# termuxinator/html5-canvas-raytracer

Measured on AMD Instinct MI355X. Metric: Mpixel/s, higher is better.
Workload: dtype f64; 1 GPU; cfg3: h8 scene (8 spheres, 2 lights, depth 3, supersample 1) at 3840x2160; SCENE, CAMERA AND LAUNCH TABLE RESIDENT (a static frame rendered again and again: cold_frame / new_camera_every_step are the other cases); one launch per frame; kernel=fma

## Files before the change

html5-canvas-raytracer_amd/csrc/rt_kernel.hip:

```cpp

#include <hip/hip_runtime.h>
#include <math.h>
#include <stdint.h>

#include "rt_device.h"
#include "rt_block.h"
#include "rt_wide.h"

#ifndef RT_STRICT
#define RT_STRICT 0
#endif
#if RT_STRICT
#define RT_LAUNCH_NAME rt_launch_trace_strict
#define RT_SCRATCH_NAME rt_scratch_trace_strict
#else
#define RT_LAUNCH_NAME rt_launch_trace_fast
#define RT_SCRATCH_NAME rt_scratch_trace_fast
#endif

#ifndef RT_WAVES_PER_EU
#define RT_WAVES_PER_EU 2
#endif

#define RT_INF __builtin_inf()

namespace {

#include "rt_literal.h"
#include "rt_kernel_math.h"
#include "rt_kernel_entry.h"
#include "rt_kernel_tables.h"
#include "rt_kernel_trace.h"

#if !RT_STRICT
typedef uint32_t __attribute__((ext_vector_type(4))) rt_px4;
__device__ __forceinline__ void rt_store16(uint32_t *p, rt_px4 v, bool through) {
  if (through) asm volatile("global_store_dwordx4 %0, %1, off sc1\n\ts_nop 1" :: "v"(p), "v"(v) : "memory");
  else *(rt_px4 *)p = v;
}
template <int N>
__device__ __forceinline__ uint32_t rt_row_down(uint32_t x) { return (uint32_t)__builtin_amdgcn_update_dpp(0, (int)x, 0x100 + N, 0xf, 0xf, true); }
#endif

template <bool REFRACT, bool COUNT, bool SS2, bool GRID, bool W1 = false>
__global__ void __launch_bounds__(W1 ? 64 : RT_WG_THREADS, ((REFRACT || !GRID) ? RT_WAVES_PER_EU : (RT_WAVES_PER_EU > 5 ? RT_WAVES_PER_EU : 5))) rt_trace(const rt_launch L) {
  static_assert(!W1 || (!REFRACT && !COUNT && !RT_STRICT), "one-wave workgroups: the reflection-only product variants");
  [[maybe_unused]] constexpr uint32_t WG_WAVES = W1 ? 1u : RT_WG_THREADS / 64u;
  constexpr uint32_t KT = W1 ? 64u : RT_WG_THREADS;
  extern __shared__ double lds_raw[];
#if defined(RT_WAVE_LOG) && !RT_STRICT
  if (unsigned long long *const wl = rt_cold_args()->wave_log; wl != nullptr && (threadIdx.x & 63u) == 0u) {
    unsigned long long *q = wl + ((size_t)(blockIdx.z * gridDim.x + blockIdx.x) * WG_WAVES + (threadIdx.x >> 6)) * 4u;
    q[0] = __builtin_amdgcn_s_memrealtime();
    q[2] = (unsigned long long)__builtin_amdgcn_s_getreg((4u) | (0u << 6) | (31u << 11)) | ((unsigned long long)__builtin_amdgcn_s_getreg((20u) | (0u << 6) | (31u << 11)) << 32);
    q[3] = rt_entry_index<W1>();
  }
#endif
  const uint32_t tid = threadIdx.x;
  const uint32_t mtl_words = L.n_objects * (uint32_t)(sizeof(rt_mtl) / 8);
  const uint32_t tex_words = 16u * 2u;
  const bool cull_lds_on = (!RT_STRICT && !COUNT) ? !GRID : (L.cull_in_lds != 0u);
  const uint32_t cull_words = cull_lds_on ? L.n_objects * 4u : 0u;
  const uint32_t image_words = mtl_words + tex_words + cull_words;
  constexpr bool IMAGE_IN_LDS = RT_STRICT || COUNT || !(GRID && !REFRACT);
  const uint32_t lds_words = IMAGE_IN_LDS ? image_words : 0u;
  const double *__restrict__ image = (const double *)L.lds_image;
  typedef uint32_t __attribute__((ext_vector_type(4))) rt_u4;
  constexpr uint32_t RT_STAGE_PIECES = 3u;
  const uint32_t image_vec = image_words >> 1;
  [[maybe_unused]] rt_u4 piece[RT_STAGE_PIECES];
  [[maybe_unused]] double stage0 = 0.0;
  const auto stage_issue = [&](const uint32_t tid) __attribute__((always_inline)) {
    if constexpr (!IMAGE_IN_LDS) {
    } else if constexpr (GRID || W1) {
      const rt_u4 *__restrict__ image4 = (const rt_u4 *)L.lds_image;
#pragma unroll
      for (uint32_t i = 0; i < RT_STAGE_PIECES; i++) if (i * KT < image_vec) piece[i] = image4[tid + i * KT];
    } else {
      stage0 = (tid < image_words) ? image[tid] : 0.0;
    }
  };
  constexpr bool UNI_OK = W1 && !REFRACT && !COUNT && !RT_STRICT && !(GRID && SS2);
  if constexpr (!UNI_OK) stage_issue(tid);
  const rt_mtl *mtl = IMAGE_IN_LDS ? (const rt_mtl *)lds_raw : (const rt_mtl *)L.lds_image;
  const rt_texture_desc *tex = IMAGE_IN_LDS ? (const rt_texture_desc *)(lds_raw + mtl_words) : (const rt_texture_desc *)((const double *)L.lds_image + mtl_words);
  const rt_geom *cull_lds = (const rt_geom *)(lds_raw + mtl_words + tex_words);
  double *acc = lds_raw + lds_words + tid;
  rt_geom cull0 = rt_geom{0.0, 0.0, 0.0, 0.0};
  if (!cull_lds_on) { const uint32_t lane0 = tid & 63u; cull0 = L.cull[lane0 < L.n_loop ? lane0 : 0u]; }

  const uint32_t lane = tid & 63u;
  const rt_pixel P0 = rt_pixel_of<SS2, W1>(L, tid);
#if !RT_STRICT
  if constexpr (W1 && !REFRACT && !COUNT && !GRID) rt_head_batch(L);
  if (P0.rows_valid == 0u) return;
#endif
  [[maybe_unused]] bool uni_try = false;
  [[maybe_unused]] uint32_t cell = 0u;
  if constexpr (UNI_OK) {
    uni_try = !P0.sky && (P0.cand >> 16) == 1u;
    if constexpr (!GRID) cell = (P0.cell >> rt_wave_of<W1>(tid)) & 0x11u;
#ifdef RT_TESTING
    if (L.no_uniform) uni_try = false;
    if (L.no_cells) cell = 0u;
#endif
    if (!uni_try && !P0.sky) stage_issue(tid);
  }
  double rgb[3];
// ... 31 lines not shown
  const auto stage_finish = [&](const uint32_t tid) __attribute__((always_inline)) {
    if constexpr (!IMAGE_IN_LDS) {
    } else if constexpr (GRID || W1) {
      rt_u4 *lds4 = (rt_u4 *)lds_raw;
      const rt_u4 *__restrict__ image4 = (const rt_u4 *)L.lds_image;
#pragma unroll
      for (uint32_t i = 0; i < RT_STAGE_PIECES; i++) {
        const uint32_t k = tid + i * KT;
        if (i * KT < image_vec && k < image_vec) lds4[k] = piece[i];
      }
      for (uint32_t k = tid + RT_STAGE_PIECES * KT; k < image_vec; k += KT) lds4[k] = image4[k];
    } else {
      if (tid < image_words) lds_raw[tid] = stage0;
      for (uint32_t k = tid + RT_WG_THREADS; k < image_words; k += RT_WG_THREADS) lds_raw[k] = image[k];
    }
  };
  [[maybe_unused]] bool uni_done = false;
  if constexpr (UNI_OK) {
    if (uni_try) {
      uni_done = trace_pixel<REFRACT, COUNT, GRID, SS2, false, W1, true>(L, (const rt_mtl *)L.lds_image, (const rt_texture_desc *)((const double *)L.lds_image + mtl_words), acc,
                                                                         cull_lds, cull0, lane, 0.0, 0.0, 0.0, 0.0, o, ray, rgb, cnt, is_probe, P0.cand | (cell << 24));
      if (!uni_done) {
        uint32_t tid4 = threadIdx.x;
        asm volatile("" : "+v"(tid4));
        stage_issue(tid4);
        stage_finish(tid4);
      }
#ifdef RT_TESTING
      else if (lane == 0u && L.uniform_waves != nullptr) {
        atomicAdd(L.uniform_waves, 1ull);
        if (cell & 1u) atomicAdd(L.uniform_waves + 1, 1ull);
      }
#endif
    }
  }
  if (!uni_done) {
    if (!UNI_OK || !uni_try) stage_finish(tid);
    if constexpr (IMAGE_IN_LDS) __syncthreads();

    const double bw = SS2 ? 15.0 : 7.0, bh = SS2 ? 3.0 : 7.0;
    const double lx = SS2 ? (double)(2u * ((lane >> 2) & 7u) + (sub & 1u)) : (double)(lane & 7u);
    const double ly = SS2 ? (double)(2u * (lane >> 5) + (sub >> 1)) : (double)(lane >> 3);
    double blk_x0 = 0.0, blk_x1 = 0.0, blk_y0 = 0.0, blk_y1 = 0.0;
    if (!UNI_OK || !uni_try) { blk_x0 = d0 - lx; blk_x1 = blk_x0 + bw; blk_y1 = d1 + ly; blk_y0 = blk_y1 - bh; }
    trace_pixel<REFRACT, COUNT, GRID, SS2, false, W1>(L, mtl, tex, acc, cull_lds, cull0, lane, blk_x0, blk_x1, blk_y0, blk_y1, o, ray, rgb, cnt, is_probe, P0.cand);
  }
  }

  uint32_t tid2 = threadIdx.x;
  asm volatile("" : "+v"(tid2));
  const rt_pixel P1 = rt_pixel_of<SS2, W1>(L, tid2);
#if !RT_STRICT
  const uint32_t wide = rt_cold_args()->wide_stores;
  asm volatile("" :: "s"(wide), "s"(L.scatter), "s"(L.rgb24), "s"(L.w), "s"(L.out), "s"(L.frame_stride));
#endif
  const uint32_t frame_i = blockIdx.z;
  const bool valid = P1.valid;
  const uint32_t r8 = to_byte(rgb[0]), g8 = to_byte(rgb[1]), b8 = to_byte(rgb[2]);
#if RT_STRICT
  uint32_t *__restrict__ out = L.scatter ? L.out_frames[frame_i] : L.out + (size_t)frame_i * L.frame_stride;
  const uint32_t orow = L.scatter ? P1.frow : P1.lrow;
#endif
  uint32_t rgbw;
  if (!SS2) rgbw = r8 | (g8 << 8) | (b8 << 16);
  else {
    uint32_t packed = r8 | (g8 << 10) | (b8 << 20);
    packed += __shfl_xor(packed, 1);
    packed += __shfl_xor(packed, 2);
    rgbw = (((packed & 1023u) + 2u) >> 2) | ((((packed >> 10) & 1023u) + 2u) >> 2 << 8) | ((((packed >> 20) & 1023u) + 2u) >> 2 << 16);
  }
#if RT_STRICT
  const uint32_t n_run = 1u;
// ... 258 lines not shown
```

html5-canvas-raytracer_amd/csrc/rt_kernel_entry.h:

```cpp

struct rt_pixel { uint32_t px, trow, frow, lrow, sub, rows_valid, run, cand, cell; bool valid, sky; };
template <bool W1>
__device__ __forceinline__ uint32_t rt_entry_slot(const rt_launch &L) {
  return (blockIdx.x & 7u) * L.order_n8 + (blockIdx.x >> (W1 ? 5 : 3));
}
template <bool W1>
__device__ __forceinline__ uint32_t rt_entry_index() { return W1 ? (((blockIdx.x >> 5) << 3) | (blockIdx.x & 7u)) : blockIdx.x; }
template <bool W1>
__device__ __forceinline__ uint32_t rt_wave_of(uint32_t tid) { return W1 ? ((blockIdx.x >> 3) & 3u) : tid >> 6; }

#if RT_STRICT
template <bool SS2, bool W1 = false>
__device__ __forceinline__ rt_pixel rt_pixel_of(const rt_launch &L, uint32_t tid) {
  const uint32_t wave = tid >> 6, lane = tid & 63u;
  const uint32_t tile_x = blockIdx.x, by = blockIdx.y;
  uint32_t tile_i, row_block;
  if (L.n_tiles == 1u) { tile_i = 0u; row_block = by; }
  else if (L.rb_shift != ~0u) { tile_i = by >> L.rb_shift; row_block = by & ((1u << L.rb_shift) - 1u); }
  else { tile_i = by / L.rb_per_tile; row_block = by - tile_i * L.rb_per_tile; }
  rt_pixel P;
  P.sub = 0u;
  if (!SS2) { P.px = tile_x * RT_TILE_W + wave * 8u + (lane & 7u); P.trow = row_block * RT_TILE_H + (lane >> 3); }
  else { const uint32_t q = lane >> 2; P.sub = lane & 3u; P.px = tile_x * RT_TILE_W + wave * 8u + (q & 7u); P.trow = row_block * 2u + (q >> 3); }
  P.frow = (L.tile_first + tile_i * L.tile_stride) * L.tile_rows + P.trow;
  P.lrow = tile_i * L.tile_rows + P.trow;
  P.valid = (P.px < L.w) && (P.trow < L.tile_rows) && (P.frow < L.h);
  P.rows_valid = 0u;
  P.sky = false; P.run = 1u; P.cand = 0u; P.cell = 0u;
  return P;
}
#else
template <bool SS2, bool W1 = false>
// ... 69 lines not shown
```

html5-canvas-raytracer_amd/csrc/rt_kernel_trace.h:

```cpp

#define RT_PIN() asm volatile("")
#define RT_ROOT(TCA, DISC)                                                                    \
        const double thc_ = rt_sqrt_nn<REFRACT>(DISC);                                                 \
        const double t0_ = (TCA) - thc_, t1_ = (TCA) + thc_;                                  \
        const bool in_ = (t0_ < eps);                                                         \
        const double t_ = in_ ? t1_ : t0_;
#define RT_CAND(IDX, TCA, DISC)                                                               \
      if (!((DISC) < 0.0)) {                                                                  \
        RT_PIN();                                                                             \
        RT_ROOT(TCA, DISC)                                                                    \
        const bool closer_ = (t_ < ht) && !(t_ < eps);              \
        ht = closer_ ? t_ : ht;                                                               \
        hcode = closer_ ? ((int)(2u * (IDX)) + (in_ ? 1 : 0)) : hcode;                        \
      }
#define RT_GENERIC(IDX, G)                                                                    \
      {                                                                                       \
        const v3 Lv_ = mk((G).ox - p.x, (G).oy - p.y, (G).oz - p.z);                          \
        const double tca_ = dot(d, Lv_);                                                      \
        const double disc_ = (G).r2 - (dot(Lv_, Lv_) - tca_ * tca_);                          \
        RT_CAND(IDX, tca_, disc_)                                                             \
      }
#define RT_ANCHORED_DISC(G)                                                                   \
        const double tca_ = d.x * (G).ox + d.y * (G).oy + d.z * (G).oz;                       \
        const double disc_ = __builtin_fma(tca_, tca_, -(G).r2);
// ... 31 lines not shown
          if (!UNI && near_) {                                                                                  \
            RT_PIN();                                                                                             \
            iu = (uint32_t)(XU); iv = (uint32_t)(XV);                    \
            const rt_launch __attribute__((address_space(4))) *K = rt_cold_args();                                \
             \
            float q_here = RT_Q_GET(level);                                                                        \
            if (rt_lvl(level) == 0 && q_here == 0.f) {                   \
              const float ex = (float)(h.x - K->cam_origin[0]), ey = (float)(h.y - K->cam_origin[1]), ez = (float)(h.z - K->cam_origin[2]);   \
              q_here = RT_Q_OF(0.f, __builtin_sqrtf(ex * ex + ey * ey + ez * ez), (float)m.inv_r, __builtin_fabsf((float)dot(d, n)), 0.f);       \
            }                                                                                                     \
            double tol = (K->mark_flags & RT_MARK_ALL) ? 2.0 : K->flag_tol * (double)fmaxf(1.f, q_here * (1.f / RT_Q_FLAT));   \
                          \
            if ((K->mark_flags & (RT_MARK_WEIGHT | RT_MARK_ALL)) == RT_MARK_WEIGHT) {                              \
              double S_ = map_valid ? acc[0] : 1.0;                                                               \
              if constexpr (FOLD_FORWARD && REFRACT) for (int i_ = 0; i_ < sp; i_++) S_ *= (parked[i_].map_valid ? parked[i_].S : 1.0) * parked[i_].a3;   \
              if (__builtin_fabs(S_) * 510.0 < 0.9) tol = -1.0;                                                    \
            }                                                                                                     \
             \
            const bool zf = !(K->mark_flags & RT_MARK_ZERO);                                                       \
            const bool bu = (zf && (FU) == 0.0 && (XU) == 0.0) || (__builtin_fabs((XU) - __builtin_rint(XU)) >= tol);    \
            const bool bv = (zf && (FV) == 0.0 && (XV) == 0.0) || (__builtin_fabs((XV) - __builtin_rint(XV)) >= tol);    \
            if (!(bu & bv)) {                                                                                      \
              uint32_t t3 = threadIdx.x;                                                                          \
              asm volatile("" : "+v"(t3));                                                                        \
              rt_mark_append<SS2>(rt_pixel_of<SS2, W1>(L, t3));                                                        \
            }                                                                                                     \
          }
#endif

#if !RT_STRICT
#define RT_SDISC(G, TC, DISC)                                                                 \
            const double TC = -(sv.x * (G).ox + sv.y * (G).oy + sv.z * (G).oz);               \
            const double DISC = __builtin_fma(TC, TC, -(G).r2);
#define RT_SROOTS(TC, THC, T0, T1) const double T0 = llen - (TC + THC), T1 = llen - (TC - THC);
#else
#define RT_SDISC(G, TC, DISC)                                                                 \
            const v3 Lv_ = mk((G).ox - h.x, (G).oy - h.y, (G).oz - h.z);                      \
            const double TC = dot(sv, Lv_);                                                   \
            const double DISC = (G).r2 - (dot(Lv_, Lv_) - TC * TC);
#define RT_SROOTS(TC, THC, T0, T1) const double T0 = TC - THC, T1 = TC + THC;
#endif
#define RT_SHADOW(J, G)                                                                       \
            {                                                                                 \
              const bool other_ = ((int)(J) != hi);                                           \
              if (COUNT && other_ && !blocked) tests++;                                       \
              RT_SDISC(G, tc_, disc_)                                                         \
// ... 24 lines not shown
                  li = (oa4_ != 0.0) ? rt_div(li, oa4_) : 0.0;                              \
                }                                                                           \
              }                                                                             \
            }

template <bool REFRACT, bool COUNT, bool GRID, bool SS2, bool ITEM = false, bool W1 = false, bool UNI = false>
__device__ __forceinline__ bool trace_pixel(const rt_launch &L, const rt_mtl *mtl, const rt_texture_desc *tex,
                                            [[maybe_unused]] double *acc, [[maybe_unused]] const rt_geom *cull_lds, [[maybe_unused]] const rt_geom cull0, [[maybe_unused]] uint32_t lane,
                                            [[maybe_unused]] double blk_x0, [[maybe_unused]] double blk_x1, [[maybe_unused]] double blk_y0,
                                            [[maybe_unused]] double blk_y1, v3 p, v3 d, double rgb[3], uint32_t cnt[3],
                                            [[maybe_unused]] bool is_probe, [[maybe_unused]] uint32_t cand_host,
                                            [[maybe_unused]] uint32_t own_sx = 0u, [[maybe_unused]] uint32_t own_sy = 0u, [[maybe_unused]] uint32_t own_f = 0u) {
  static_assert(!UNI || (W1 && !REFRACT && !COUNT && !ITEM && !RT_STRICT), "uniform-material path: the one-wave-workgroup product kernels");
#ifdef RT_TESTING
  uint32_t probe_n = 0;
  double probe_li = 0.0;
#endif
  const sphere_kptr objs = (sphere_kptr)L.objects;
  const geom_kptr geom = (geom_kptr)L.geom;
  const uint32_t N = L.n_objects, NL = L.n_lights;
  const double eps = L.epsilon;
  const uint32_t NLOOP = L.n_loop;
  const uint32_t enc = L.enclosing;
  const bool cull_lds_on = (!RT_STRICT && !COUNT) ? !GRID : (L.cull_in_lds != 0u);
#if RT_STRICT
  constexpr bool FOLD_FORWARD = false;
#else
  constexpr bool FOLD_FORWARD = true;
#endif
  constexpr bool LEAN = !RT_STRICT && !REFRACT && !COUNT && !ITEM;
  [[maybe_unused]] frame<REFRACT> stack[FOLD_FORWARD ? 1 : RT_MAX_SEGS];
  [[maybe_unused]] park parked[(FOLD_FORWARD && REFRACT) ? RT_MAX_SEGS : 1];
  [[maybe_unused]] int sp = 0;
  [[maybe_unused]] bool map_valid = false;
  int level = 0;
  [[maybe_unused]] uint32_t tree_path = 1u;
#if defined(RT_TESTING) && defined(RT_ABLATE_BOUNCE)
  uint32_t segs_left = L.segs ? 1 : 0;
#else
  uint32_t segs_left = L.segs;
#endif
  double ret[3] = {0.0, 0.0, 0.0};

  double ht = RT_INF; int hcode = -1;
  if constexpr (UNI) { if (segs_left == 0) return false; }
  if (segs_left != 0) {
        [[maybe_unused]] const geom_kptr ga = (geom_kptr)L.geom_cam;
#if !RT_STRICT
        if constexpr (UNI) {
          const uint32_t i = cand_host & 255u;
          const rt_geom g0 = rt_load_geom32(ga, i);
          typename rt_mtl_src<true>::type &mu = *rt_mtl_at<true>(mtl, i);
          if ((mu.albedo[3] > 0.0 && segs_left > 1) || rt_mtl_kind(mu) == RT_SAMPLER_STARS) return false;
          RT_ANCHORED_DISC(g0)
          const double t0_ = tca_ - rt_sqrt_nn<REFRACT>(disc_);
          const bool met_ = !(disc_ < 0.0) && (t0_ < ht) && !(t0_ < eps);
          if (__ballot(!met_) != 0ull) return false;
#if defined(RT_TESTING) && defined(RT_ABLATE_UNIFORM)
          rgb[0] = rgb[1] = rgb[2] = 0.0;
          return true;
#endif
          ht = t0_; hcode = (int)(2u * i);
        } else
        if (cand_host != 0u) {
          { const uint32_t i = cand_host & 255u; const rt_geom g0 = rt_load_geom32(ga, i); RT_ANCHORED(i, g0) }
          if (cand_host >= (2u << 16)) { const uint32_t i = (cand_host >> 8) & 255u; const rt_geom g0 = rt_load_geom32(ga, i); RT_ANCHORED(i, g0) }
        } else
#endif
        for (uint32_t base = 0; base < NLOOP; base += 64u) {
          const uint32_t j = base + lane;
          const uint32_t jj = j < NLOOP ? j : 0u;
          double c0 = cull0.ox, c1 = cull0.oy, c2 = cull0.oz, c3 = cull0.r2;
          if constexpr (ITEM) {
          } else if (cull_lds_on) {
            const rt_geom __attribute__((address_space(3))) *g = (const rt_geom __attribute__((address_space(3))) *)cull_lds + jj;
            c0 = g->ox; c1 = g->oy; c2 = g->oz; c3 = g->r2;
          } else if (base != 0u) {
            const rt_geom __attribute__((address_space(1))) *g = (const rt_geom __attribute__((address_space(1))) *)L.cull + jj;
            c0 = g->ox; c1 = g->oy; c2 = g->oz; c3 = g->r2;
          }
          const rt_geom cr = rt_geom{c0, c1, c2, c3};
          unsigned long long m = __ballot(j < NLOOP) & __ballot(cr.ox * L.proj_d <= blk_x1) & __ballot(cr.oy * L.proj_d >= blk_x0) &
                                 __ballot(cr.oz * L.proj_d <= blk_y1) & __ballot(cr.r2 * L.proj_d >= blk_y0);
          if constexpr (ITEM) m = (NLOOP - base >= 64u) ? ~0ull : ((1ull << (NLOOP - base)) - 1ull);
          while (m) {
            const uint32_t i = base + (uint32_t)__builtin_ctzll(m);
            m &= m - 1ull;
#if RT_STRICT
            const rt_geom g0 = rt_load_geom32(geom, i);
            RT_GENERIC(i, g0)
#else
            const rt_geom g0 = rt_load_geom32(ga, i);
            RT_ANCHORED(i, g0)
#endif
          }
        }
  }
  bool searched = true;
  [[maybe_unused]] bool first_bounce = false;
#if !RT_STRICT
  if (!UNI && L.sky_fast && segs_left != 0 && __ballot(hcode >= 0) == 0ull) {
    if (COUNT) { cnt[0]++; cnt[2] += N; }
    rgb[0] = L.sky_rgb[0]; rgb[1] = L.sky_rgb[1]; rgb[2] = L.sky_rgb[2];
    return true;
  }
#endif

  if (segs_left != 0) {
    for (;;) {
      if (COUNT) cnt[0]++;
      if (!UNI && !searched) {
        bool scanned = false;
#if !RT_STRICT
        if constexpr (GRID) {
          if (rt_cold_args()->bounce_table != nullptr) {
            const uint32_t from = (uint32_t)(hcode >> 1);
            const double ax = __builtin_fabs(d.x), ay = __builtin_fabs(d.y), az = __builtin_fabs(d.z);
            const bool bx = (ax >= ay) && (ax >= az), by = !bx && (ay >= az);
            const double dm = bx ? d.x : (by ? d.y : d.z);
            const double du = bx ? d.y : d.x, dv = (bx || by) ? d.z : d.y;
            const double sc = (0.5 * RT_BGRID) * __builtin_amdgcn_rcp(__builtin_fabs(dm));
            const double fu = __builtin_fmin(__builtin_fmax(__builtin_fma(du, sc, 0.5 * RT_BGRID), 0.0), (double)(RT_BGRID - 1u));
            const double fv = __builtin_fmin(__builtin_fmax(__builtin_fma(dv, sc, 0.5 * RT_BGRID), 0.0), (double)(RT_BGRID - 1u));
            const uint32_t face = (bx ? 0u : (by ? 2u : 4u)) + ((dm < 0.0) ? 1u : 0u);
            const uint32_t key = from * RT_BCELLS + face * (RT_BGRID * RT_BGRID) + (uint32_t)fv * RT_BGRID + (uint32_t)fu;
            const uint32_t words = (NLOOP + 63u) >> 6;
            ht = RT_INF; hcode = -1;
            for (uint32_t wd = 0; wd < words; wd++) {
              unsigned long long cand = 0ull, todo = __ballot(true);
              uint32_t distinct = 0;
              while (todo) {
                const uint32_t k0 = (uint32_t)__builtin_amdgcn_readlane((int)key, (int)__builtin_ctzll(todo));
// ... 78 lines not shown
      if (!UNI && hcode < 0) {
        { const auto &mc = RT_COLD(miss_color); ret[0] = mc[0]; ret[1] = mc[1]; ret[2] = mc[2]; }
#ifdef RT_TESTING
        if (is_probe && probe_n < RT_PROBE_NODES) {
          double *q = L.probe + (size_t)(probe_n++) * RT_PROBE_WORDS;
          for (uint32_t z = 0; z < RT_PROBE_WORDS; z++) q[z] = 0.0;
          q[0] = (double)(REFRACT ? tree_path : (1u << rt_lvl(level))); q[1] = -1.0; q[2] = ht; q[9] = d.x; q[10] = d.y; q[11] = d.z;
          q[17] = (double)segs_left; q[19] = p.x; q[20] = p.y; q[21] = p.z; q[23] = 1.0;
        }
#endif
      } else {
        typename rt_mtl_src<UNI>::type &m = *rt_mtl_at<UNI>(mtl, (uint32_t)hi);
        const v3 h = mk(p.x + d.x * ht, p.y + d.y * ht, p.z + d.z * ht);
#if RT_STRICT
        double nlen;
        const v3 n = unit(mk(h.x - m.origin[0], h.y - m.origin[1], h.z - m.origin[2]), &nlen);
#else
        const double inv_r = m.inv_r;
        const v3 n = mk((h.x - m.origin[0]) * inv_r, (h.y - m.origin[1]) * inv_r, (h.z - m.origin[2]) * inv_r);
#endif
        v3 l;
        if constexpr (UNI) l = n;
        else l = inside ? mk(-n.x, -n.y, -n.z) : n;
        const double a0 = m.albedo[0], a1 = m.albedo[1], a2 = m.albedo[2], a3 = m.albedo[3];
        const double a4 = REFRACT ? m.albedo[4] : 0.0;
#if !RT_STRICT && !defined(RT_ABLATE_QAMP)
        if (!UNI && (rt_lvl(level) != 0 || ((a3 > 0.0 || a4 > 0.0) && segs_left > 1))) {
          const float ir_ = (float)inv_r;
          const float q_ = RT_Q_OF(RT_Q_GET(level), (float)ht, ir_, __builtin_fabsf((float)dot(d, n)), rt_r_get(level));
          level = rt_q_put(level, q_);
          level = rt_r_put(level, __builtin_amdgcn_rcpf(ir_));
        }
#endif

        double col[3];
#if defined(RT_TESTING) && defined(RT_ABLATE_SAMPLER)
        const int kind = RT_SAMPLER_COLOR;
#else
        const int kind = rt_mtl_kind(m);
#endif
#if RT_STRICT
        if (kind == RT_SAMPLER_TEXTURE) {
          double t_at, t_as;
          rt_atan2_asin<REFRACT>(-n.z, -n.x, -n.y, &t_at, &t_as);
          const double u = RT_DIV_CONST(t_at, M_PI) / 2.0 + 0.5;
          const double v = RT_DIV_CONST(t_as, M_PI / 2.0) / 2.0 + 0.5;
          const rt_texture_desc td = rt_tex_desc<UNI>(tex, rt_mtl_texture(m));
// ... 33 lines not shown
          RT_XY_INDEX(xu, xv, 1.0, 1.0)
          const uint32_t xi = min(iu, td.width - 1u), yi = min(iv, td.height - 1u);
          const uint32_t texel = *(const uint32_t *)(rt_cold_args()->texel_base + td.texels_offset + ((size_t)yi * td.width + xi) * 4u);
          col[0] = RT_DIV_CONST((double)(texel & 255u), 255.0); col[1] = RT_DIV_CONST((double)((texel >> 8) & 255u), 255.0);
          col[2] = RT_DIV_CONST((double)((texel >> 16) & 255u), 255.0);
        } else if (kind == RT_SAMPLER_CHECKER) {
          if constexpr (!UNI) rt_atan2_asin<REFRACT>(-n.y, -n.x, -n.z, &t_at, &t_as);
          const double u = RT_DIV_CONST(t_at, M_PI) / 2.0 + 0.5;
          const double v = RT_DIV_CONST(t_as, M_PI / 2.0) / 2.0 + 0.5;
          const double xu = u * m.c[6], xv = v * m.c[7];
          RT_XY_INDEX(xu, xv, m.c[6], m.c[7])
          const int c = (int)((iu ^ iv) & 1u);
          if constexpr (UNI) {
            double k0 = m.c[0], k1 = m.c[1], k2 = m.c[2], k3 = m.c[3], k4 = m.c[4], k5 = m.c[5];
            asm volatile("" : "+s"(k0), "+s"(k1), "+s"(k2), "+s"(k3), "+s"(k4), "+s"(k5));
            col[0] = c ? k3 : k0; col[1] = c ? k4 : k1; col[2] = c ? k5 : k2;
          } else { col[0] = m.c[3 * c]; col[1] = m.c[3 * c + 1]; col[2] = m.c[3 * c + 2]; }
#endif
        } else if (!UNI && kind == RT_SAMPLER_STARS) {
          uint32_t sx = own_sx, sy = own_sy, f = own_f;
          if constexpr (!ITEM) {
            f = blockIdx.z;
            uint32_t t3 = threadIdx.x;
            asm volatile("" : "+v"(t3));
            const rt_pixel P = rt_pixel_of<SS2, W1>(L, t3);
            sx = SS2 ? 2u * P.px + (P.sub & 1u) : P.px; sy = SS2 ? 2u * P.frow + (P.sub >> 1) : P.frow;
          }
          const unsigned long long pix = (unsigned long long)sy * (SS2 ? 2u * L.w : L.w) + sx;
          const uint32_t path = REFRACT ? tree_path : (1u << rt_lvl(level));
          const rt_launch __attribute__((address_space(4))) *K = rt_cold_args();
          const uint32_t mix = lowbias32(K->stars_seed + K->stars_step * f);
          double c = star_uniform((uint32_t)pix, (uint32_t)(pix >> 32), path, mix);
          c = (c >= m.c[6]) ? 0.0 : c * m.c[7];
          col[0] = col[1] = col[2] = c;
        } else { col[0] = m.c[0]; col[1] = m.c[1]; col[2] = m.c[2]; }
#if !RT_STRICT
        }
#endif

        if constexpr (FOLD_FORWARD && REFRACT) {
#pragma unroll
          for (int c = 0; c < 3; c++) acc[(10 + c) * RT_WG_THREADS] = col[c];
        }

        double diffuse = 0.0, specular = 0.0;
        [[maybe_unused]] double draw = 0.0, sraw = 0.0;
// ... 146 lines not shown
                asm volatile("" : "+v"(off_));
                spec_m = (const rt_mtl *)((const char *)mtl + off_);
              }
              const int32_t spec_n = spec_m->spec_n;
              if (spd > 0.0) specular += rt_pow_spec<UNI>(spd, spec_n, &spec_m->specular_exponent);
#else
              if (spd > 0.0) specular += rt_pow(spd, m.specular_exponent);
#endif
            }
          }
          if constexpr (UNI) {
            draw = diffuse; sraw = specular;
            diffuse = rt_min1_nn(diffuse) * a1;
            specular = rt_min1_nn(specular) * a2;
          } else {
          diffuse = min1(diffuse) * a1;
          specular = min1(specular) * a2;
          }
#ifdef RT_TESTING
          probe_li = li;
#endif
        }

#if RT_STRICT
        const v3 nq = n;
#else
        const v3 nq = inside ? mk(-l.x, -l.y, -l.z) : l;
#endif
        v3 r = mk(0, 0, 0); double rlen = 0.0;
#if !RT_STRICT
        if constexpr (LEAN) { if (!UNI && a3 > 0.0 && segs_left > 1) r = unit_go(reflect(d, l), &rlen); } else
#endif
        if (!UNI && a3 > 0.0 && segs_left > 1) r = unit(reflect(d, nq), &rlen);
        v3 f = mk(0, 0, 0); double flen = 0.0;
        if (REFRACT && a4 > 0.0 && segs_left > 1) {
          const double dn = dot(d, nq);
          double cosi = -((dn < -1.0) ? -1.0 : min1(dn));
          v3 nn = nq; double eta;
          if (cosi < 0.0) { cosi = -cosi; nn = mk(-nq.x, -nq.y, -nq.z); eta = m.refract_index; }
          else eta = rt_rcp(m.refract_index);
          const double k = 1.0 - eta * eta * (1.0 - cosi * cosi);
          if (k > 0.0) {
            const double q = eta * cosi - rt_sqrt(k);
            f = mk(d.x * eta + nn.x * q, d.y * eta + nn.y * q, d.z * eta + nn.z * q);
          } else f = reflect(d, nn);
          f = unit(f, &flen);
// ... 124 lines not shown
              for (int c = 0; c < 3; c++) {
                acc[(1 + c) * T] = pk.ds[c] + ret[c] * pk.a3; acc[(4 + c) * T] = pk.amb[c]; acc[(7 + c) * T] = __builtin_fmax(pk.amb[c], 1.0);
              }
            } else {
              const double S = pk.S;
#pragma unroll
              for (int c = 0; c < 3; c++) {
                const double Dn = pk.ds[c] + ret[c] * pk.a3;
                const double l2 = __builtin_fma(S, pk.amb[c], pk.O[c]), h2 = __builtin_fma(S, __builtin_fmax(pk.amb[c], 1.0), pk.O[c]);
                acc[(1 + c) * T] = __builtin_fma(S, Dn, pk.O[c]);
                acc[(4 + c) * T] = __builtin_fmax(pk.LO[c], __builtin_fmin(pk.HI[c], l2));
                acc[(7 + c) * T] = __builtin_fmax(pk.LO[c], __builtin_fmin(pk.HI[c], h2));
              }
              acc[0] = S * coef;
            }
            map_valid = true;
            p = mk(pk.h[0], pk.h[1], pk.h[2]); d = mk(pk.f[0], pk.f[1], pk.f[2]);
            tree_path = 2u * pk.path + 1u; segs_left = pk.segs_left - 1u; level = pk.level + 1;
            hcode = pk.hcode;

            resumed = true;
          }
        }
        if (!resumed) break;
      } else {
        bool resumed = false;
        while (level > 0) {
          level--; segs_left++; tree_path >>= 1;
          frame<REFRACT> &fr = stack[level];
          if constexpr (REFRACT) {
            if (fr.phase == 0) {
              fr.re[0] = ret[0] * fr.a3; fr.re[1] = ret[1] * fr.a3; fr.re[2] = ret[2] * fr.a3;
              if (fr.has_f) {
                fr.phase = 1;
                p = mk(fr.h[0], fr.h[1], fr.h[2]); d = mk(fr.f[0], fr.f[1], fr.f[2]);
                tree_path = 2u * tree_path + 1u;
                level++; segs_left--;
                resumed = true;
                break;
              }
#pragma unroll
              for (int c = 0; c < 3; c++) ret[c] = maxa(fr.amb[c], min1(fr.ds[c] + fr.re[c]));
            } else {
#pragma unroll
              for (int c = 0; c < 3; c++) ret[c] = maxa(fr.amb[c], min1(fr.ds[c] + fr.re[c] + ret[c] * fr.a4));
            }
          } else {
#pragma unroll
            for (int c = 0; c < 3; c++) ret[c] = maxa(fr.amb[c], min1(fr.ds[c] + ret[c] * fr.a3));
          }
        }
        if (!resumed) break;
      }
    }
  }
  rgb[0] = ret[0]; rgb[1] = ret[1]; rgb[2] = ret[2];
  return true;
}

#undef RT_Q_GET
#undef RT_Q_OF
#undef RT_ROOT
#undef RT_CAND
#undef RT_GENERIC
#undef RT_ANCHORED_DISC
#undef RT_ANCHORED
#undef RT_XY_INDEX
#undef RT_SDISC
#undef RT_SROOTS
#undef RT_SHADOW
#undef RT_SHADOW_U
```

html5-canvas-raytracer_amd/csrc/rt_launch.hip:

```cpp

#include "rt_api_internal.h"

extern "C" int rt_render_tiles_device(rt_scene_dev *s, uint32_t w, uint32_t h, const rt_tiles *tiles, void *d_out, void *hip_stream,
                                      uint32_t flags, rt_stats *stats) {
  return rt_render_batch_device(s, w, h, tiles, 1u, d_out, 0u, hip_stream, flags, stats);
}

namespace {
int render_batch_impl(rt_scene_dev *s, uint32_t w, uint32_t h, const rt_tiles *tiles, uint32_t n_frames, void *d_out, uint64_t frame_stride_bytes,
                      void *const *d_frames, void *hip_stream, uint32_t flags, rt_stats *stats, uint32_t ss_override = 0u);
#ifdef RT_TESTING
thread_local struct { double *d_buf; uint32_t x, y; } g_probe = {nullptr, 0u, 0u};
#endif

void bind_scene_order(const rt_scene_dev *s, rt_launch &K) {
  const uint8_t *ob = obj_block(s);
  K.objects = (const rt_sphere *)(ob + s->o_objs);
  K.geom = (const rt_geom *)(ob + s->o_geom);
  K.lds_image = lds_image_of(s);
  K.n_loop = s->hd.n_objects;
  K.enclosing = ~0u;
  memcpy(K.miss_color, s->hd.miss_color, sizeof K.miss_color);
}
}
// ... 205 lines not shown
}

struct colour_call {
  rt_scene_dev *s; device_state &D; hipStream_t stream;
  uint32_t w, h, ss; const rt_tiles *tiles; uint32_t n_frames, flags;
  bool ss2, count, compact;
  test_switches t;
};
struct retrace_result {
  const uint32_t *marks_read = nullptr; uint32_t marks_read_slot = 0;
  uint64_t centre_items = 0;
  bool retraced_all = false, strict_rendered = false;
};
struct marks_guard {
  rt_scene_dev::mark_state temp = {~0u, nullptr, device_mem(), nullptr, 0u};
  ~marks_guard() { if (temp.d_marks.h) (void)hipStreamSynchronize(temp.stream); }
};

int launched(int err) { return err != 0 ? fail(RT_ERR_DEVICE, "kernel launch: %s", hipGetErrorString((hipError_t)err)) : RT_OK; }

unsigned lds_for(const rt_scene_dev *s, rt_trace_variant v, unsigned lds_pad) {
  if (v.strict) return s->lds_bytes + lds_pad + RT_WG_THREADS * 8u;
  const unsigned fold = (v.refract ? 13u : 10u) * (v.one_wave ? 64u : RT_WG_THREADS) * 8u;
  return ((v.grid && !v.refract) ? 0u : s->lds_bytes) + lds_pad + fold;
}

void bind_kernel(const rt_scene_dev *s, rt_launch &K, bool plain, const test_switches &t) {
  const rt_scene_header &hd = s->hd;
  const bool order_b = s->has_b && !plain;
  const uint8_t *ob = obj_block(s);
  if (order_b) {
    K.objects = (const rt_sphere *)(ob + s->o_objs_b);
    K.geom = (const rt_geom *)(ob + s->o_geom) + (size_t)hd.n_objects * (1 + hd.n_lights);
    K.lds_image = lds_image_of(s) + s->lds_image_bytes;
    K.n_loop = K.enclosing = hd.n_objects - 1;
    memcpy(K.miss_color, hd.miss_color, sizeof K.miss_color);
  } else bind_scene_order(s, K);
  const rt_geom *gc = (const rt_geom *)cam_block(s) + (order_b ? 2 * (size_t)hd.n_objects : 0);
  K.geom_cam = gc;
  K.cull = gc + hd.n_objects;
  K.geom_light = K.geom + hd.n_objects;
  K.shadow_grid = (!plain && !t.no_grid && s->has_sg) ? ob + s->o_sg : nullptr;
  K.bounce_table = (!plain && !t.no_bounce && s->has_bt) ? ob + s->o_bt : nullptr;
  K.enclosing_flat = (order_b && s->enclosing_flat) ? 1u : 0u;
  K.cull_in_lds = s->cull_in_lds ? 1u : 0u;
  K.sky_fast = (!plain && sky_fast(s)) ? 1u : 0u;
// ... 217 lines not shown
    rc = strict_main ? strict_launch(c, L, c.count) : product_launch(c, L, temp_marks, o);
  }
  if (rc) return rc;

  if ((rc = clock.finish(stats, stats ? tile_set_pixels(w, h, tiles) * n_frames : 0u))) return rc;
  if (stats) {
    if (c.count) {
      unsigned long long n[3];
      HIP_TRY(hipMemcpy(n, D.d_counters, sizeof n, hipMemcpyDeviceToHost));
      stats->rays = n[0]; stats->shadow_rays = n[1]; stats->sphere_tests = n[2];
    }
    if (o.strict_rendered) stats->exact_samples = stats->pixels;
    if (o.marks_read) {
      uint32_t n_marked = 0;
      HIP_TRY(hipMemcpy(&n_marked, o.marks_read + o.marks_read_slot, sizeof n_marked, hipMemcpyDeviceToHost));
      stats->exact_samples = (n_marked > RT_MARKS_CAP || o.retraced_all) ? stats->pixels : n_marked + o.centre_items;
    }
    stats->total_ms = clock.host_ms();
  }
  return RT_OK;
}
}

extern "C" size_t rt_adaptive_work_bytes(uint32_t w, uint32_t h) {
  return (w == 0 || h == 0 || w > 65536u / 2u || h > 65536u / 2u) ? 0 : (size_t)rt_adaptive_bytes(w, h);
}

#ifdef RT_TESTING
extern "C" int rt_test_adaptive_mask(const uint8_t *rgba, uint32_t w, uint32_t h, uint32_t threshold, uint8_t *mask_out) {
  if (!rgba || !mask_out || w == 0 || h == 0 || threshold > 256u) return fail(RT_ERR_INVALID, "rt_test_adaptive_mask: NULL argument, empty frame or threshold above 256");
  const auto at = [&](uint32_t x, uint32_t y) { uint32_t v; memcpy(&v, rgba + ((size_t)y * w + x) * 4u, 4u); return v; };
  for (uint32_t y = 0; y < h; y++)
    for (uint32_t x = 0; x < w; x++) {
      const uint32_t c = at(x, y);
      mask_out[(size_t)y * w + x] = rt_adaptive_refines(c, x > 0u ? at(x - 1u, y) : c, x + 1u < w ? at(x + 1u, y) : c, y > 0u ? at(x, y - 1u) : c,
                                                        y + 1u < h ? at(x, y + 1u) : c, threshold) ? 1u : 0u;
    }
  return RT_OK;
}
extern "C" uint32_t rt_test_adaptive_box(uint32_t sum, uint32_t k) { return rt_adaptive_box(sum, k); }
extern "C" uint32_t rt_test_adaptive_refine_grid(uint32_t w, uint32_t h, uint32_t k) { return rt_adaptive_refine_grid(w, h, k); }
#endif

namespace {
int adaptive_scratch(bool refract, uint32_t k, size_t *out) {
  static std::mutex mu;
// ... 371 lines not shown
```

html5-canvas-raytracer_amd/rt_host.py:

```python
import base64
import ctypes as C
import json
import numbers
import os
import struct

HERE = os.path.dirname(os.path.abspath(__file__))
ROOT = os.path.dirname(HERE)
SCENES_DIR = os.path.join(HERE, "scenes")
LIB_PATH = os.environ.get("RT_HIP_LIB") or os.path.join(HERE, "csrc", "librt_hip.so")
TEST_LIB_PATH = os.path.join(HERE, "csrc", "librt_hip_test.so")

RT_SCENE_MAGIC = 0x31535452
RT_ABI_VERSION = 2
HEADER_BYTES, SPHERE_BYTES, TEXDESC_BYTES = 208, 192, 16
SAMPLER_COLOR, SAMPLER_TEXTURE, SAMPLER_CHECKER, SAMPLER_STARS = 0, 1, 2, 3

RT_FLAG_COUNT = 1
RT_FLAG_STRICT_FP = 2
RT_FLAG_RGB24 = 4
RT_FLAG_NO_SKY = 8
RT_FLAG_SKY_ONLY = 16
RT_FLAG_COMPACT = 32
RT_FLAG_STARS_PER_FRAME = 64
# ... 178 lines not shown


class RtLightingOutputs(C.Structure):
    _fields_ = [("diffuse", C.c_void_p), ("intensity", C.c_void_p), ("lit", C.c_void_p), ("rgba", C.c_void_p)]


ABI = {
    "rt_init": (C.c_int, [C.c_int]),
    "rt_shutdown": (None, []),
    "rt_device_count": (C.c_int, []),
    "rt_last_error": (C.c_char_p, []),
    "rt_abi_version": (C.c_uint32, []),
    "rt_build_id": (C.c_char_p, []),
    "rt_elapsed_report": (C.c_int, [C.c_void_p, C.c_char_p, C.c_size_t]),
    "rt_scene_validate": (C.c_int, [C.c_void_p, C.c_size_t]),
    "rt_scene_cull_rects": (C.c_int, [C.c_void_p, C.c_size_t, C.POINTER(C.c_double)]),
    "rt_scene_bounce_candidates": (C.c_int, [C.c_void_p, C.c_size_t, C.c_uint32, C.POINTER(C.c_double), C.POINTER(C.c_uint64)]),
    "rt_scene_launch_table": (C.c_int, [C.c_void_p, C.c_size_t, C.c_uint32, C.c_uint32, C.POINTER(RtTiles), C.c_int, C.POINTER(C.c_uint32),
                                        C.POINTER(C.c_uint32), C.POINTER(C.c_uint32)]),
    "rt_scene_upload": (C.c_int, [C.c_int, C.c_void_p, C.c_size_t, C.POINTER(C.c_void_p)]),
    "rt_scene_free": (None, [C.c_void_p]),
    "rt_scene_set_camera": (C.c_int, [C.c_void_p, C.POINTER(C.c_double), C.POINTER(C.c_double), C.POINTER(C.c_double), C.POINTER(C.c_double), C.c_void_p]),
    "rt_scene_set_stars_seed": (C.c_int, [C.c_void_p, C.c_uint32]),
    "rt_scene_set_objects": (C.c_int, [C.c_void_p, C.c_uint32, C.c_uint32, C.c_void_p, C.c_void_p]),
    "rt_scene_set_lights": (C.c_int, [C.c_void_p, C.c_uint32, C.c_uint32, C.POINTER(C.c_double), C.c_void_p]),
    "rt_scene_set_light_intensity": (C.c_int, [C.c_void_p, C.c_double]),
    "rt_scene_set_texels": (C.c_int, [C.c_void_p, C.c_uint32, C.c_uint32, C.c_uint32, C.c_uint32, C.c_uint32, C.c_void_p, C.c_size_t, C.c_void_p]),
    "rt_scene_set_texels_device": (C.c_int, [C.c_void_p, C.c_uint32, C.c_uint32, C.c_uint32, C.c_uint32, C.c_uint32, C.c_void_p, C.c_size_t, C.c_void_p]),
    "rt_render_tiles_device": (C.c_int, [C.c_void_p, C.c_uint32, C.c_uint32, C.POINTER(RtTiles), C.c_void_p, C.c_void_p,
                                         C.c_uint32, C.POINTER(RtStats)]),
    "rt_render_batch_device": (C.c_int, [C.c_void_p, C.c_uint32, C.c_uint32, C.POINTER(RtTiles), C.c_uint32, C.c_void_p, C.c_uint64,
                                         C.c_void_p, C.c_uint32, C.POINTER(RtStats)]),
    "rt_render": (C.c_int, [C.c_void_p, C.c_size_t, C.c_uint32, C.c_uint32, C.c_void_p, C.c_uint32, C.POINTER(RtStats)]),
    "rt_render_progressive": (C.c_int, [C.c_void_p, C.c_size_t, C.c_uint32, C.c_uint32, C.c_void_p, C.c_uint32, C.c_void_p, C.c_void_p, C.c_uint32,
                                        C.POINTER(RtStats)]),
    "rt_render_options": (C.c_int, [C.c_int, C.c_uint32]),
    "rt_alloc_pinned": (C.c_void_p, [C.c_size_t]),
    "rt_free_pinned": (None, [C.c_void_p]),
    "rt_alloc_device": (C.c_void_p, [C.c_int, C.c_size_t]),
    "rt_free_device": (None, [C.c_int, C.c_void_p]),
    "rt_copy_to_host": (C.c_int, [C.c_int, C.c_void_p, C.c_void_p, C.c_size_t]),
    "rt_deinterleave_device": (C.c_int, [C.c_int, C.c_void_p, C.c_void_p, C.c_uint32, C.c_uint32, C.c_uint32, C.c_uint32,
                                         C.c_uint64, C.c_void_p]),
    "rt_memset_device": (C.c_int, [C.c_int, C.c_void_p, C.c_int, C.c_size_t]),
    "rt_render_scatter_device": (C.c_int, [C.c_void_p, C.c_uint32, C.c_uint32, C.POINTER(RtTiles), C.c_uint32, C.POINTER(C.c_void_p), C.c_void_p,
                                           C.c_uint32, C.POINTER(RtStats)]),
# ... 142 lines not shown

class Renderer:

    def __init__(self, scene, device=0, lib=None):
        self.lib = lib or load_library()
        self.blob = scene if isinstance(scene, (bytes, bytearray)) else flatten_scene(scene)
        self.device = device
        if self.lib.rt_device_count() < 0:
            _check(self.lib, self.lib.rt_init(0), "rt_init")
        h = C.c_void_p()
        buf = C.create_string_buffer(self.blob, len(self.blob))
        _check(self.lib, self.lib.rt_scene_upload(device, buf, len(self.blob), C.byref(h)), "rt_scene_upload")
        self.handle = h

    def set_camera(self, camera, stream=None):
        v = [(C.c_double * 3)(*camera[k]) for k in ("origin", "axisX", "axisY", "axisZ")]
        _check(self.lib, self.lib.rt_scene_set_camera(self.handle, v[0], v[1], v[2], v[3], C.c_void_p(stream or 0)), "rt_scene_set_camera")

    def set_stars_seed(self, seed):
        if not (isinstance(seed, int) and not isinstance(seed, bool) and 0 <= seed < 2 ** 32):
            raise ValueError("stars seed must be an integer in [0, 2^32)")
        _check(self.lib, self.lib.rt_scene_set_stars_seed(self.handle, seed), "rt_scene_set_stars_seed")

    def set_objects(self, objects, first=0, stream=None):
        recs = bytes(objects) if isinstance(objects, (bytes, bytearray)) else sphere_records(objects)
        if len(recs) % SPHERE_BYTES:
            raise ValueError("sphere records are %d bytes each" % SPHERE_BYTES)
        buf = C.create_string_buffer(recs, max(len(recs), 1))
        _check(self.lib, self.lib.rt_scene_set_objects(self.handle, first, len(recs) // SPHERE_BYTES, buf, C.c_void_p(stream or 0)),
               "rt_scene_set_objects")

    def set_lights(self, lights, first=0, stream=None):
        flat = light_positions(lights)
        if isinstance(first, bool) or not isinstance(first, int) or first < 0:
            raise ValueError("first must be a light index")
        xyz = (C.c_double * max(len(flat), 1))(*flat)
        _check(self.lib, self.lib.rt_scene_set_lights(self.handle, first, len(flat) // 3, xyz, C.c_void_p(stream or 0)), "rt_scene_set_lights")

    def set_light_intensity(self, value):
        if isinstance(value, bool) or not isinstance(value, numbers.Real):
            raise ValueError("light intensity must be a number")
        _check(self.lib, self.lib.rt_scene_set_light_intensity(self.handle, float(value)), "rt_scene_set_light_intensity")

    def texture_size(self, texture):
        n_textures, = struct.unpack_from("<I", self.blob, 176)
        tex_off, = struct.unpack_from("<Q", self.blob, 200)
# ... 1113 lines not shown
```

include/rt_hip.h:

```cpp
#ifndef RT_HIP_H
#define RT_HIP_H

#include <stddef.h>
#include <stdint.h>

#ifdef __cplusplus
extern "C" {
#endif

#define RT_ABI_VERSION 2u
#define RT_SCENE_MAGIC 0x31535452u
#define RT_REFERENCE_BUILD "741"
#define RT_LIBRARY_REVISION "r4"

#define RT_MAX_OBJECTS  256u
#define RT_MAX_LIGHTS   16u
#define RT_MAX_TEXTURES 16u
#define RT_MAX_SEGS     16u

typedef enum rt_status {
  RT_OK = 0,
  RT_ERR_INVALID = -1,
  RT_ERR_UNSUPPORTED = -2,
  RT_ERR_DEVICE = -3,
// ... 85 lines not shown
void rt_shutdown(void);
int rt_device_count(void);
const char *rt_last_error(void);
uint32_t rt_abi_version(void);
const char *rt_build_id(void);

int rt_scene_validate(const void *scene_blob, size_t blob_bytes);

int rt_scene_cull_rects(const void *scene_blob, size_t blob_bytes, double *out_4n);

int rt_scene_bounce_candidates(const void *scene_blob, size_t blob_bytes, uint32_t from, const double dir[3], uint64_t *out_words);

int rt_scene_launch_table(const void *scene_blob, size_t blob_bytes, uint32_t w, uint32_t h, const rt_tiles *tiles, int ranked,
                          uint32_t *out_entries, uint32_t *n_workgroups, uint32_t *n_blocks);

int rt_scene_upload(int device, const void *scene_blob, size_t blob_bytes, rt_scene_dev **out);
void rt_scene_free(rt_scene_dev *scene);

int rt_scene_set_camera(rt_scene_dev *scene, const double origin[3], const double axis_x[3], const double axis_y[3], const double axis_z[3],
                        void *hip_stream);

int rt_scene_set_stars_seed(rt_scene_dev *scene, uint32_t seed);

int rt_scene_set_objects(rt_scene_dev *scene, uint32_t first, uint32_t count, const rt_sphere *records, void *hip_stream);

int rt_scene_set_lights(rt_scene_dev *scene, uint32_t first, uint32_t count, const double *xyz, void *hip_stream);

int rt_scene_set_light_intensity(rt_scene_dev *scene, double light_intensity);

int rt_scene_set_texels(rt_scene_dev *scene, uint32_t texture, uint32_t x, uint32_t y, uint32_t w, uint32_t h, const void *rgba,
                        size_t pitch_bytes, void *hip_stream);
int rt_scene_set_texels_device(rt_scene_dev *scene, uint32_t texture, uint32_t x, uint32_t y, uint32_t w, uint32_t h, const void *d_rgba,
                               size_t pitch_bytes, void *hip_stream);

int rt_render_tiles_device(rt_scene_dev *scene, uint32_t w, uint32_t h, const rt_tiles *tiles,
                           void *d_out_rgba, void *hip_stream, uint32_t flags, rt_stats *stats);

int rt_render_batch_device(rt_scene_dev *scene, uint32_t w, uint32_t h, const rt_tiles *tiles, uint32_t n_frames,
                           void *d_out_rgba, uint64_t frame_stride_bytes, void *hip_stream, uint32_t flags, rt_stats *stats);

int rt_render_scatter_device(rt_scene_dev *scene, uint32_t w, uint32_t h, const rt_tiles *tiles, uint32_t n_frames,
                             void *const *d_frames, void *hip_stream, uint32_t flags, rt_stats *stats);

#define RT_IPC_HANDLE_BYTES 64u
int rt_ipc_export(int device, const void *d_ptr, void *handle_out);
int rt_ipc_open(int device, const void *handle, void **d_ptr_out);
// ... 294 lines not shown
```

Measured before the change: 159,900 Mpixel/s.

## Raise occupancy of one-wave non-grid trace variant by trimming LDS and registers

For one-wave non-grid kernels, the launch bound rises to at least six waves per EU, and only the material table is staged in LDS. Textures and cull rectangles are now read from global memory instead. The lane index is recomputed with mbcnt rather than kept live, and the return color is parked in LDS across the bounce loop. Albedo values are reloaded after the loop to shorten register live ranges. An occupancy query API is added for inspection. The trade is more global and LDS traffic and reloads in exchange for fewer VGPRs and LDS bytes per workgroup, if the W1 path is the one in use.

```diff
diff --git a/html5-canvas-raytracer_amd/csrc/rt_kernel.hip b/html5-canvas-raytracer_amd/csrc/rt_kernel.hip
--- a/html5-canvas-raytracer_amd/csrc/rt_kernel.hip
+++ b/html5-canvas-raytracer_amd/csrc/rt_kernel.hip
@@ -21,6 +21,12 @@
 #ifndef RT_WAVES_PER_EU
 #define RT_WAVES_PER_EU 2
 #endif
+
+constexpr unsigned rt_waves_per_eu(bool refract, bool grid, bool w1) {
+  return (w1 && !grid && !refract) ? (RT_WAVES_PER_EU > 6 ? RT_WAVES_PER_EU : 6)
+       : (refract || !grid)        ? RT_WAVES_PER_EU
+                                   : (RT_WAVES_PER_EU > 5 ? RT_WAVES_PER_EU : 5);
+}
 
 #define RT_INF __builtin_inf()
 
@@ -43,7 +49,7 @@
 #endif
 
 template <bool REFRACT, bool COUNT, bool SS2, bool GRID, bool W1 = false>
-__global__ void __launch_bounds__(W1 ? 64 : RT_WG_THREADS, ((REFRACT || !GRID) ? RT_WAVES_PER_EU : (RT_WAVES_PER_EU > 5 ? RT_WAVES_PER_EU : 5))) rt_trace(const rt_launch L) {
+__global__ void __launch_bounds__(W1 ? 64 : RT_WG_THREADS, rt_waves_per_eu(REFRACT, GRID, W1)) rt_trace(const rt_launch L) {
   static_assert(!W1 || (!REFRACT && !COUNT && !RT_STRICT), "one-wave workgroups: the reflection-only product variants");
   [[maybe_unused]] constexpr uint32_t WG_WAVES = W1 ? 1u : RT_WG_THREADS / 64u;
   constexpr uint32_t KT = W1 ? 64u : RT_WG_THREADS;
@@ -61,7 +67,8 @@
   const uint32_t tex_words = 16u * 2u;
   const bool cull_lds_on = (!RT_STRICT && !COUNT) ? !GRID : (L.cull_in_lds != 0u);
   const uint32_t cull_words = cull_lds_on ? L.n_objects * 4u : 0u;
-  const uint32_t image_words = mtl_words + tex_words + cull_words;
+  constexpr bool MTL_ONLY = W1 && !GRID;
+  const uint32_t image_words = MTL_ONLY ? mtl_words : mtl_words + tex_words + cull_words;
   constexpr bool IMAGE_IN_LDS = RT_STRICT || COUNT || !(GRID && !REFRACT);
   const uint32_t lds_words = IMAGE_IN_LDS ? image_words : 0u;
   const double *__restrict__ image = (const double *)L.lds_image;
@@ -83,7 +90,7 @@
   constexpr bool UNI_OK = W1 && !REFRACT && !COUNT && !RT_STRICT && !(GRID && SS2);
   if constexpr (!UNI_OK) stage_issue(tid);
   const rt_mtl *mtl = IMAGE_IN_LDS ? (const rt_mtl *)lds_raw : (const rt_mtl *)L.lds_image;
-  const rt_texture_desc *tex = IMAGE_IN_LDS ? (const rt_texture_desc *)(lds_raw + mtl_words) : (const rt_texture_desc *)((const double *)L.lds_image + mtl_words);
+  const rt_texture_desc *tex = (IMAGE_IN_LDS && !MTL_ONLY) ? (const rt_texture_desc *)(lds_raw + mtl_words) : (const rt_texture_desc *)((const double *)L.lds_image + mtl_words);
   const rt_geom *cull_lds = (const rt_geom *)(lds_raw + mtl_words + tex_words);
   double *acc = lds_raw + lds_words + tid;
   rt_geom cull0 = rt_geom{0.0, 0.0, 0.0, 0.0};
@@ -161,6 +168,7 @@
                                                                          cull_lds, cull0, lane, 0.0, 0.0, 0.0, 0.0, o, ray, rgb, cnt, is_probe, P0.cand | (cell << 24));
       if (!uni_done) {
         uint32_t tid4 = threadIdx.x;
+        if constexpr (MTL_ONLY) tid4 = rt_lane_again(); else
         asm volatile("" : "+v"(tid4));
         stage_issue(tid4);
         stage_finish(tid4);
@@ -187,6 +195,7 @@
   }
 
   uint32_t tid2 = threadIdx.x;
+  if constexpr (W1 && !GRID) tid2 = rt_lane_again(); else
   asm volatile("" : "+v"(tid2));
   const rt_pixel P1 = rt_pixel_of<SS2, W1>(L, tid2);
 #if !RT_STRICT
diff --git a/html5-canvas-raytracer_amd/csrc/rt_kernel_entry.h b/html5-canvas-raytracer_amd/csrc/rt_kernel_entry.h
--- a/html5-canvas-raytracer_amd/csrc/rt_kernel_entry.h
+++ b/html5-canvas-raytracer_amd/csrc/rt_kernel_entry.h
@@ -8,6 +8,12 @@
 __device__ __forceinline__ uint32_t rt_entry_index() { return W1 ? (((blockIdx.x >> 5) << 3) | (blockIdx.x & 7u)) : blockIdx.x; }
 template <bool W1>
 __device__ __forceinline__ uint32_t rt_wave_of(uint32_t tid) { return W1 ? ((blockIdx.x >> 3) & 3u) : tid >> 6; }
+
+__device__ __forceinline__ uint32_t rt_lane_again() {
+  uint32_t x;
+  asm volatile("v_mbcnt_lo_u32_b32 %0, -1, 0\n\tv_mbcnt_hi_u32_b32 %0, -1, %0" : "=v"(x));
+  return x;
+}
 
 #if RT_STRICT
 template <bool SS2, bool W1 = false>
diff --git a/html5-canvas-raytracer_amd/csrc/rt_kernel_trace.h b/html5-canvas-raytracer_amd/csrc/rt_kernel_trace.h
--- a/html5-canvas-raytracer_amd/csrc/rt_kernel_trace.h
+++ b/html5-canvas-raytracer_amd/csrc/rt_kernel_trace.h
@@ -77,6 +77,7 @@
             const bool bv = (zf && (FV) == 0.0 && (XV) == 0.0) || (__builtin_fabs((XV) - __builtin_rint(XV)) >= tol);    \
             if (!(bu & bv)) {                                                                                      \
               uint32_t t3 = threadIdx.x;                                                                          \
+              if constexpr (W1 && !GRID) t3 = rt_lane_again(); else                                               \
               asm volatile("" : "+v"(t3));                                                                        \
               rt_mark_append<SS2>(rt_pixel_of<SS2, W1>(L, t3));                                                        \
             }                                                                                                     \
@@ -147,7 +148,7 @@
   const double eps = L.epsilon;
   const uint32_t NLOOP = L.n_loop;
   const uint32_t enc = L.enclosing;
-  const bool cull_lds_on = (!RT_STRICT && !COUNT) ? !GRID : (L.cull_in_lds != 0u);
+  const bool cull_lds_on = (!RT_STRICT && !COUNT) ? (!GRID && !W1) : (L.cull_in_lds != 0u);
 #if RT_STRICT
   constexpr bool FOLD_FORWARD = false;
 #else
@@ -166,6 +167,7 @@
   uint32_t segs_left = L.segs;
 #endif
   double ret[3] = {0.0, 0.0, 0.0};
+  constexpr bool PARK_RET = FOLD_FORWARD && W1 && !GRID && !REFRACT && !COUNT && !ITEM && !UNI;
 
   double ht = RT_INF; int hcode = -1;
   if constexpr (UNI) { if (segs_left == 0) return false; }
@@ -200,7 +202,7 @@
           } else if (cull_lds_on) {
             const rt_geom __attribute__((address_space(3))) *g = (const rt_geom __attribute__((address_space(3))) *)cull_lds + jj;
             c0 = g->ox; c1 = g->oy; c2 = g->oz; c3 = g->r2;
-          } else if (base != 0u) {
+          } else if (base != 0u || (W1 && !GRID)) {
             const rt_geom __attribute__((address_space(1))) *g = (const rt_geom __attribute__((address_space(1))) *)L.cull + jj;
             c0 = g->ox; c1 = g->oy; c2 = g->oz; c3 = g->r2;
           }
@@ -233,6 +235,7 @@
 
   if (segs_left != 0) {
     for (;;) {
+      if constexpr (PARK_RET) ret[0] = ret[1] = ret[2] = 0.0;
       if (COUNT) cnt[0]++;
       if (!UNI && !searched) {
         bool scanned = false;
@@ -357,7 +360,9 @@
         v3 l;
         if constexpr (UNI) l = n;
         else l = inside ? mk(-n.x, -n.y, -n.z) : n;
-        const double a0 = m.albedo[0], a1 = m.albedo[1], a2 = m.albedo[2], a3 = m.albedo[3];
+        double a0 = m.albedo[0];
+        const double a1 = m.albedo[1], a2 = m.albedo[2];
+        double a3 = m.albedo[3];
         const double a4 = REFRACT ? m.albedo[4] : 0.0;
 #if !RT_STRICT && !defined(RT_ABLATE_QAMP)
         if (!UNI && (rt_lvl(level) != 0 || ((a3 > 0.0 || a4 > 0.0) && segs_left > 1))) {
@@ -437,6 +442,7 @@
           if constexpr (!ITEM) {
             f = blockIdx.z;
             uint32_t t3 = threadIdx.x;
+            if constexpr (W1 && !GRID) t3 = rt_lane_again(); else
             asm volatile("" : "+v"(t3));
             const rt_pixel P = rt_pixel_of<SS2, W1>(L, t3);
             sx = SS2 ? 2u * P.px + (P.sub & 1u) : P.px; sy = SS2 ? 2u * P.frow + (P.sub >> 1) : P.frow;
@@ -629,6 +635,13 @@
 #endif
         }
 
+        if constexpr (PARK_RET) {
+          uint32_t hi2 = (uint32_t)hi;
+          asm volatile("" : "+v"(hi2));
+          const rt_mtl &m2 = *rt_mtl_at<false>(mtl, hi2);
+          a0 = m2.albedo[0]; a3 = m2.albedo[3];
+        }
+
 #if RT_STRICT
         const v3 nq = n;
 #else
@@ -799,7 +812,15 @@
             resumed = true;
           }
         }
-        if (!resumed) break;
+        if (!resumed) {
+          if constexpr (PARK_RET) {
+#pragma unroll
+            for (int c = 0; c < 3; c++) acc[(1 + c) * T] = ret[c];
+            uint32_t fin = 1u;
+            asm volatile("" : "+v"(fin));
+            if (fin != 0u) break;
+          } else break;
+        }
       } else {
         bool resumed = false;
         while (level > 0) {
@@ -830,6 +851,10 @@
         if (!resumed) break;
       }
     }
+    if constexpr (PARK_RET) {
+#pragma unroll
+      for (int c = 0; c < 3; c++) ret[c] = acc[(1 + c) * 64u];
+    }
   }
   rgb[0] = ret[0]; rgb[1] = ret[1]; rgb[2] = ret[2];
   return true;
diff --git a/html5-canvas-raytracer_amd/csrc/rt_launch.hip b/html5-canvas-raytracer_amd/csrc/rt_launch.hip
--- a/html5-canvas-raytracer_amd/csrc/rt_launch.hip
+++ b/html5-canvas-raytracer_amd/csrc/rt_launch.hip
@@ -251,6 +251,7 @@
 unsigned lds_for(const rt_scene_dev *s, rt_trace_variant v, unsigned lds_pad) {
   if (v.strict) return s->lds_bytes + lds_pad + RT_WG_THREADS * 8u;
   const unsigned fold = (v.refract ? 13u : 10u) * (v.one_wave ? 64u : RT_WG_THREADS) * 8u;
+  if (v.one_wave && !v.grid) return s->hd.n_objects * (unsigned)sizeof(rt_mtl) + lds_pad + fold;
   return ((v.grid && !v.refract) ? 0u : s->lds_bytes) + lds_pad + fold;
 }
 
@@ -514,6 +515,23 @@
 }
 }
 
+extern "C" int rt_scene_trace_occupancy(rt_scene_dev *s, int four_waves, int *out_workgroups_per_cu, uint32_t *out_lds_bytes) {
+  if (!s || !out_workgroups_per_cu) return fail(RT_ERR_INVALID, "rt_scene_trace_occupancy: NULL argument");
+  if (int rc = ensure_device(s->device)) return rc;
+  HIP_TRY(hipSetDevice(G.dev[s->device].hip_id));
+  const uint32_t ss = s->hd.supersample;
+  if (ss > 2u) return fail(RT_ERR_UNSUPPORTED, "rt_scene_trace_occupancy: supersample %u renders on the sample grid", ss);
+  const rt_trace_variant v = rt_trace_variant_of(strict_scene(s), false, s->refract, false, ss == 2u, s->cull_in_lds, false, four_waves != 0);
+  const void *f = (v.strict ? rt_kernel_trace_strict : rt_kernel_trace_fast)(v);
+  if (!f) return fail(RT_ERR_DEVICE, "rt_scene_trace_occupancy: no kernel for the variant");
+  const unsigned lds = lds_for(s, v, 0u);
+  int n = 0;
+  HIP_TRY(hipOccupancyMaxActiveBlocksPerMultiprocessor(&n, f, v.one_wave ? 64 : (int)RT_WG_THREADS, lds));
+  *out_workgroups_per_cu = n;
+  if (out_lds_bytes) *out_lds_bytes = lds;
+  return RT_OK;
+}
+
 extern "C" size_t rt_adaptive_work_bytes(uint32_t w, uint32_t h) {
   return (w == 0 || h == 0 || w > 65536u / 2u || h > 65536u / 2u) ? 0 : (size_t)rt_adaptive_bytes(w, h);
 }
diff --git a/html5-canvas-raytracer_amd/rt_host.py b/html5-canvas-raytracer_amd/rt_host.py
--- a/html5-canvas-raytracer_amd/rt_host.py
+++ b/html5-canvas-raytracer_amd/rt_host.py
@@ -224,6 +224,7 @@
     "rt_scene_free": (None, [C.c_void_p]),
     "rt_scene_set_camera": (C.c_int, [C.c_void_p, C.POINTER(C.c_double), C.POINTER(C.c_double), C.POINTER(C.c_double), C.POINTER(C.c_double), C.c_void_p]),
     "rt_scene_set_stars_seed": (C.c_int, [C.c_void_p, C.c_uint32]),
+    "rt_scene_trace_occupancy": (C.c_int, [C.c_void_p, C.c_int, C.POINTER(C.c_int), C.POINTER(C.c_uint32)]),
     "rt_scene_set_objects": (C.c_int, [C.c_void_p, C.c_uint32, C.c_uint32, C.c_void_p, C.c_void_p]),
     "rt_scene_set_lights": (C.c_int, [C.c_void_p, C.c_uint32, C.c_uint32, C.POINTER(C.c_double), C.c_void_p]),
     "rt_scene_set_light_intensity": (C.c_int, [C.c_void_p, C.c_double]),
@@ -412,6 +413,11 @@
             raise ValueError("stars seed must be an integer in [0, 2^32)")
         _check(self.lib, self.lib.rt_scene_set_stars_seed(self.handle, seed), "rt_scene_set_stars_seed")
 
+    def trace_occupancy(self, four_waves=False):
+        n, lds = C.c_int(), C.c_uint32()
+        _check(self.lib, self.lib.rt_scene_trace_occupancy(self.handle, 1 if four_waves else 0, C.byref(n), C.byref(lds)), "rt_scene_trace_occupancy")
+        return n.value, lds.value
+
     def set_objects(self, objects, first=0, stream=None):
         recs = bytes(objects) if isinstance(objects, (bytes, bytearray)) else sphere_records(objects)
         if len(recs) % SPHERE_BYTES:
diff --git a/include/rt_hip.h b/include/rt_hip.h
--- a/include/rt_hip.h
+++ b/include/rt_hip.h
@@ -131,6 +131,8 @@
 
 int rt_scene_set_stars_seed(rt_scene_dev *scene, uint32_t seed);
 
+int rt_scene_trace_occupancy(rt_scene_dev *scene, int four_waves, int *out_workgroups_per_cu, uint32_t *out_lds_bytes);
+
 int rt_scene_set_objects(rt_scene_dev *scene, uint32_t first, uint32_t count, const rt_sphere *records, void *hip_stream);
 
 int rt_scene_set_lights(rt_scene_dev *scene, uint32_t first, uint32_t count, const double *xyz, void *hip_stream);
```

Measured after the change: 168,700 Mpixel/s (median of 6 runs). +5.5%, better.
